# Azure/mmlspark

Hardware: AMD Instinct MI355X
Metric: lightgbm_train_rows_per_sec (higher is better)
Workload: dtype fp32; 1 GPU; model=LightGBMClassifier, rows_per_gpu=10000000, features=100, num_leaves=63, max_bin=255, objective=binary, global_batch=10000000, parallelism=dp1, sync=single rank, categorical=0, matrix=dense

## Files before the change

### mmlspark_amd/models/gbdt/trainer.py

```python
from __future__ import annotations

import heapq
import math
import os
import time
from dataclasses import dataclass, field
from typing import Dict, List, Optional

import numpy as np
import torch

from ...ops import backend
from ...parallel.comm import Comm
from .binning import BinMapper
from .booster import Booster
from .objectives import Objective
from .tree import Tree

NEG_INF = float("-inf")


@dataclass
class TrainConfig:
    num_iterations: int = 100
# ... 231 lines not shown
            order = np.lexsort((present, ratio))
            GL = np.cumsum(g[order], dtype=np.float32)
            HL = np.cumsum(hh[order], dtype=np.float32)
            CL = np.cumsum(c[order], dtype=np.float32)
            G, H, C = GL[-1], HL[-1], CL[-1]

            def sc(Gs, Hs):
                Ga = np.maximum(np.abs(Gs) - np.float32(cfg.lambda_l1),
                                np.float32(0))
                return Ga * Ga / (Hs + np.float32(cfg.lambda_l2)
                                  + np.float32(1e-32))

            gain = sc(GL, HL) + sc(G - GL, H - HL) - sc(
                np.float32(G), np.float32(H))
            valid = ((CL >= cfg.min_data_in_leaf)
                     & (C - CL >= cfg.min_data_in_leaf)
                     & (HL >= cfg.min_sum_hessian_in_leaf)
                     & (H - HL >= cfg.min_sum_hessian_in_leaf))
            gain = np.where(valid, gain, np.float32(NEG_INF))
            gain[-1] = NEG_INF
            k = int(gain.argmax())
            bg = float(gain[k])
            if not np.isfinite(bg):
                continue
            if best is None or bg > best[0]:
                cats = present[order[: k + 1]].tolist()
                best = [bg, int(f), 0, float(GL[k]), float(HL[k]),
                        float(CL[k]), cats]
        return best

    def _best_split(self, hist, feat_mask):
        return self._scan(hist.unsqueeze(0), feat_mask)[0]

    def _partition(self, leaf) -> tuple:
        t0 = time.perf_counter()
        if leaf.cats is not None:
            gq, j = leaf.feat // 4, leaf.feat % 4
            bins = self.binned[gq, leaf.rows.long(), j]
            cats_t = torch.tensor(leaf.cats, dtype=bins.dtype,
                                  device=bins.device)
            mask = torch.isin(bins, cats_t)
            rows_l, rows_r = leaf.rows[mask], leaf.rows[~mask]
        else:
            known = (int(leaf.CL) if (self.fixed
                                      and not self.comm.is_distributed
                                      and leaf.C < 1.6e7)
                     else -1)
            rows_l, rows_r = backend.partition_rows(
                self.binned, leaf.rows, leaf.feat, leaf.bin,
                known_left=known)
        self.stats.partition_s += time.perf_counter() - t0
        return rows_l, rows_r

    def _grow_native(self, rows_root, grad, hess, feat_mask):
        from ...ops import _hip_grower
        cfg = self.cfg
        pg = self.comm.native_group()
        cats_active = [f for f in self.cat_features
                       if feat_mask is None or bool(feat_mask[f])]
        num_mask = feat_mask
        if self.cat_features:
            num_mask = (feat_mask.clone() if feat_mask is not None else
                        torch.ones(self.nf_pad, dtype=torch.bool,
                                   device=self.device))
            num_mask[self.cat_features] = False
        cats_t = (torch.tensor(cats_active, dtype=torch.int64)
                  if cats_active else None)
        t0 = time.perf_counter()
        d = _hip_grower.grow_tree_native(
            self.binned, self.binned_pair, rows_root.contiguous(), grad, hess,
            cfg.max_bin,
            self.nf, self.scale_g, self.scale_h, cfg.lambda_l1, cfg.lambda_l2,
            float(cfg.min_data_in_leaf), cfg.min_sum_hessian_in_leaf,
            cfg.min_gain_to_split, cfg.max_delta_step, cfg.num_leaves,
            cfg.max_depth, num_mask, cats_t, self.cat_smooth, pg,
            self.comm.is_distributed or bool(os.environ.get(
                "MMLSPARK_AMD_FORCE_DIST_GROWER")))
        self.stats.hist_s += time.perf_counter() - t0
        feature = d["feature"].numpy()
        thr_bin = d["thr_bin"].numpy()
        cat_offset = d["cat_offset"].numpy()
        threshold = np.array(
            [float("nan") if cat_offset[i] >= 0 else
             self.bin_mapper.bin_upper_value(int(f), int(b)) if f >= 0 else 0.0
             for i, (f, b) in enumerate(zip(feature, thr_bin))],
            dtype=np.float32)
        tree = Tree(feature, threshold, thr_bin, d["left"].numpy(),
                    d["right"].numpy(), d["value"].numpy(),
                    d["count"].numpy(), d["gain"].numpy(),
                    d["leaf_index"].numpy(), shrinkage=1.0,
                    cat_offset=cat_offset,
                    cat_words=d["cat_words"].numpy().view(np.uint32))
        offs = d["leaf_offsets"].tolist()
        nodes = d["leaf_nodes"].tolist()
        leaves = []
        for i, nid in enumerate(nodes):
            lf = _Leaf(int(nid), d["leaf_rows"][offs[i]:offs[i + 1]], None,
                       0, 0, 0, 0)
            leaves.append(lf)
        self.native_leaves = (d["leaf_rows"], d["leaf_offsets"], nodes)
        return tree, leaves

    native_ok = True
    native_leaves = None

    def grow(self, rows_root: torch.Tensor, grad: torch.Tensor,
             hess: torch.Tensor, feat_mask) -> (Tree, List):
        self.native_leaves = None
        if (self.native_ok and self.fixed and not self.voting
                and not os.environ.get(
                    "MMLSPARK_AMD_NO_NATIVE_GROWER")):
            try:
                from ...ops import _hip_grower
                self.set_scales(grad, hess)
                return self._grow_native(rows_root, grad, hess, feat_mask)
            except ImportError:
                pass
        cfg = self.cfg
        feature, threshold, thr_bin = [], [], []
        left, right, value, count, gain_arr, leaf_idx = [], [], [], [], [], []
        cat_off, cat_words = [], []

        def new_node():
            feature.append(-1)
            threshold.append(0.0)
            thr_bin.append(0)
            left.append(-1)
            right.append(-1)
            value.append(0.0)
            count.append(0.0)
            gain_arr.append(0.0)
            leaf_idx.append(-1)
            cat_off.append(-1)
            return len(feature) - 1

        self.set_scales(grad, hess)
        root_hist = self._hist(rows_root, grad, hess)
        if self.voting:
            t = torch.stack([grad[rows_root.long()].sum(),
                             hess[rows_root.long()].sum(),
                             torch.tensor(float(rows_root.numel()),
                                          device=self.device)])
            self.comm.all_reduce(t)
            G, H, C = float(t[0]), float(t[1]), float(t[2])
        else:
            G, H, C = self._sums(root_hist)
        root = _Leaf(new_node(), rows_root, root_hist, G, H, C, 0)
        (root.gain, root.feat, root.bin, root.GL, root.HL, root.CL,
         root.cats) = self._best_split(root_hist, feat_mask)
        count[root.node_id] = C
        value[root.node_id] = _leaf_output(G, H, cfg)

        heap = [(-root.gain, 0, root)]
        seq = 1
        n_leaves = 1
        final_leaves = [root]

        while n_leaves < cfg.num_leaves and heap:
            ngain, _, leaf = heapq.heappop(heap)
            if -ngain <= cfg.min_gain_to_split or not np.isfinite(-ngain):
                continue
            if cfg.max_depth > 0 and leaf.depth >= cfg.max_depth:
                continue
            final_leaves.remove(leaf)

            rows_l, rows_r = self._partition(leaf)

            GL, HL, CL = leaf.GL, leaf.HL, leaf.CL
# ... 196 lines not shown
            objective.group_sizes = group_sizes

        from .sparse import CsrMatrix, bin_csr, fit_bin_mapper_csr
        self.is_sparse = isinstance(X, CsrMatrix)
        if self.is_sparse:
            if cfg.categorical_features:
                raise ValueError("categorical features need dense input "
                                 "(set matrixType='dense')")
            if cfg.boosting == "dart":
                raise ValueError("dart boosting needs dense input "
                                 "(set matrixType='dense')")
        if binned_cache is not None:
            self.bin_mapper, self.binned = binned_cache
        elif self.is_sparse:
            self.bin_mapper = fit_bin_mapper_csr(
                X, n_bins=cfg.max_bin, comm=comm, seed=cfg.seed,
                sample_size=cfg.bin_sample_count)
            self.binned = bin_csr(X, self.bin_mapper)
        else:
            self.bin_mapper = BinMapper.fit(X, n_bins=cfg.max_bin, comm=comm,
                                            seed=cfg.seed,
                                            sample_size=cfg.bin_sample_count,
                                            categorical=cfg.categorical_features,
                                            max_bin_by_feature=cfg.max_bin_by_feature)
            self.binned = self.bin_mapper.transform(X)

        device, n, K = self.device, self.n, self.K
        if init_booster is not None and init_booster.trees:
            base = torch.from_numpy(init_booster.base_score).to(device)
            self.preds = init_booster.predict_raw(X)
            self.trees: List[Tree] = list(init_booster.trees)
            self.tree_w: List[float] = list(init_booster.tree_weights)
        else:
            base = self._global_init_score()
            if base.numel() < K:
                base = base.expand(K).contiguous()
            self.preds = base.unsqueeze(0).expand(n, K).clone()
            if init_score is not None:
                sc = init_score.to(device).float()
                self.preds += sc.unsqueeze(-1) if sc.dim() == 1 else sc
            self.trees = []
            self.tree_w = []
        self.base = base
        n_global = n
        if comm.is_distributed:
            t = torch.tensor([float(n)], device=device)
            comm.all_reduce(t)
            n_global = int(t[0])
        grower_cls = SparseTreeGrower if self.is_sparse else TreeGrower
        self.grower = grower_cls(self.binned, self.nf, cfg, comm, self.stats,
                                 self.bin_mapper, n_global=n_global)
        self.gen = torch.Generator(device="cpu")
        self.all_rows = torch.arange(n, dtype=torch.int32, device=device)
        self.n_start_trees = len(self.trees)
        self.it = 0

    def _global_init_score(self):
        y, weight, device = self.y, self.weight, self.device
        obj, comm = self.objective, self.comm
        if not self.cfg.boost_from_average:
            return torch.zeros(1, device=device)
        if comm.is_distributed:
            w = weight if weight is not None else torch.ones_like(
                y, dtype=torch.float32)
            sums = torch.stack([(y.float() * w).sum(), w.sum()]).to(device)
            comm.all_reduce(sums)
            mean = sums[0] / sums[1].clamp_min(1e-12)
            if obj.name == "binary":
                p = mean.clamp(1e-6, 1 - 1e-6)
                sig = getattr(obj, "sigmoid", 1.0)
                return (torch.log(p / (1 - p)) / sig).reshape(1)
            if obj.name in ("regression", "regression_l2"):
                return mean.reshape(1)
            if obj.name in ("poisson", "tweedie"):
                return torch.log(mean.clamp_min(1e-8)).reshape(1)
            s0 = obj.init_score(y, weight).to(device).float()
            comm.all_reduce(s0)
            return s0 / comm.world_size
        return obj.init_score(y, weight).to(device)

    def step(self):
        cfg, gen, K, device = self.cfg, self.gen, self.K, self.device
        trees, tree_w, preds = self.trees, self.tree_w, self.preds
        it = self.it
        rf_mode = cfg.boosting == "rf"
        dart_mode = cfg.boosting == "dart"
        goss_mode = cfg.boosting == "goss"

        t0 = time.perf_counter()
        dropped = []
        if dart_mode and trees[self.n_start_trees:]:
            gen.manual_seed(cfg.seed * 7919 + it)
            if float(torch.rand(1, generator=gen)) >= cfg.skip_drop:
                cand = list(range(self.n_start_trees, len(trees)))
                if cfg.uniform_drop:
                    pdrop = torch.full((len(cand),), cfg.drop_rate)
                else:
                    tw = torch.tensor([abs(tree_w[t]) for t in cand])
                    pdrop = (cfg.drop_rate * len(cand)
                             * tw / tw.sum().clamp_min(1e-12)).clamp(0, 1)
                mask = torch.rand(len(cand), generator=gen) < pdrop
                dropped = [cand[i] for i in range(len(cand)) if bool(mask[i])]
                dropped = dropped[: cfg.max_drop]
        if dropped:
            drop_contrib = torch.zeros_like(preds)
            for t in dropped:
                k = (t - self.n_start_trees) % K
                drop_contrib[:, k] += tree_w[t] * predict_tree_binned(
                    trees[t], self.binned, device)
            preds_used = preds - drop_contrib
        else:
            preds_used = preds
        if rf_mode:
            preds_used = self.base.unsqueeze(0).expand(self.n, K)
        grad, hess = self.objective.grad_hess(preds_used, self.y, self.weight)
        self.stats.grad_s += time.perf_counter() - t0

        gen.manual_seed(cfg.bagging_seed * 104729 + it * 31 + self.comm.rank)
        if goss_mode and it >= 1:
            rows_root = _goss_sample(grad, hess, cfg, gen)
        elif (cfg.pos_bagging_fraction < 1.0 or cfg.neg_bagging_fraction < 1.0) \
                and cfg.bagging_freq > 0 and it % cfg.bagging_freq == 0:
            pos = (self.y > 0).cpu()
            keep = torch.rand(self.n, generator=gen) < torch.where(
                pos, torch.tensor(cfg.pos_bagging_fraction),
                torch.tensor(cfg.neg_bagging_fraction))
            rows_root = keep.nonzero(as_tuple=True)[0].to(
                device, torch.int32).sort().values
            if rows_root.numel() == 0:
                rows_root = self.all_rows
        elif (cfg.bagging_freq > 0 and cfg.bagging_fraction < 1.0
              and it % cfg.bagging_freq == 0) or rf_mode:
            frac = cfg.bagging_fraction if cfg.bagging_fraction < 1.0 else 0.632
            m = max(1, int(frac * self.n))
            perm = torch.randperm(self.n, generator=gen)[:m].to(device)
            rows_root = perm.to(torch.int32).sort().values
        else:
            rows_root = self.all_rows

        feat_mask = None
        if cfg.feature_fraction < 1.0:
            gen_f = torch.Generator(device="cpu")
            gen_f.manual_seed(cfg.seed * 524287 + it)
            kf = max(1, int(cfg.feature_fraction * self.nf))
            sel = torch.randperm(self.nf, generator=gen_f)[:kf]
            feat_mask = torch.zeros(self.grower.nf_pad, dtype=torch.bool,
                                    device=device)
            feat_mask[sel.to(device)] = True

        new_trees = []
        for k in range(K):
            tree, leaves = self.grower.grow(rows_root, grad[:, k].contiguous(),
                                            hess[:, k].contiguous(), feat_mask)
            tree.shrinkage = 1.0 if rf_mode else cfg.learning_rate
            if not rf_mode:
                t0 = time.perf_counter()
                live = [lf for lf in leaves if lf.rows.numel()]
                native = self.grower.native_leaves
                if (native is not None and not dropped
                        and preds.is_cuda and preds.dtype == torch.float32):
                    from ...ops import _hip_grower
                    leaf_rows, leaf_offsets, nodes = native
                    vals = torch.tensor(
                        [float(tree.value[nid]) * tree.shrinkage
                         for nid in nodes], dtype=torch.float32,
                        device=device)
                    _hip_grower.apply_leaf_values(preds[:, k], leaf_rows,
                                                  leaf_offsets, vals)
                elif live:
                    all_rows = torch.cat([lf.rows for lf in live]).long()
                    sizes = [lf.rows.numel() for lf in live]
                    vals = torch.tensor(
                        [float(tree.value[lf.node_id]) * tree.shrinkage
                         for lf in live], device=device)
                    expanded = torch.repeat_interleave(
                        vals, torch.tensor(sizes, device=device))
                    preds[:, k].index_add_(0, all_rows, expanded)
                self.stats.partition_s += time.perf_counter() - t0
            new_trees.append(tree)

        if dropped:
            kdrop = len(dropped)
            if cfg.xgboost_dart_mode:
                factor = kdrop / (kdrop + cfg.learning_rate)
                new_scale = cfg.learning_rate / (kdrop + cfg.learning_rate)
            else:
                factor = kdrop / (kdrop + 1.0)
                new_scale = 1.0 / (kdrop + 1.0)
            for t in dropped:
                k = (t - self.n_start_trees) % K
                delta = (factor - 1.0) * tree_w[t]
                preds[:, k] += delta * predict_tree_binned(trees[t], self.binned,
                                                           device)
                tree_w[t] *= factor
            for k, tr in enumerate(new_trees):
                excess = (1.0 - new_scale) * tr.shrinkage
                preds[:, k] -= excess * predict_tree_binned(tr, self.binned, device)
                tr.shrinkage *= new_scale

        for tr in new_trees:
            trees.append(tr)
            tree_w.append(1.0)
        self.stats.iterations += 1
        self.it += 1

    def booster(self) -> Booster:
        tw = list(self.tree_w)
        if self.cfg.boosting == "rf" and self.stats.iterations:
            tw = [1.0 / self.stats.iterations] * len(tw)
        return Booster(list(self.trees), self.objective.name, self.K,
                       self.base.cpu().numpy(), self.nf, self.feature_names,
                       self.bin_mapper,
                       sigmoid=getattr(self.objective, "sigmoid", 1.0),
# ... 103 lines not shown
```

### mmlspark_amd/ops/hip/gbdt_grower.cpp

```cpp
#include <torch/extension.h>
#include <torch/csrc/distributed/c10d/ProcessGroup.hpp>
#include <c10/hip/HIPGuard.h>
#include <c10/hip/HIPStream.h>
#include <hip/hip_runtime.h>

#include <algorithm>
#include <cmath>
#include <cstdlib>
#include <memory>
#include <mutex>
#include <numeric>
#include <queue>
#include <vector>

extern "C" {
void launch_arena_gather(const void*, long, const float*, const float*,
                         const int*, long, int, double, double, void*, void*,
                         int*, hipStream_t);
void launch_partition_arena(const void*, const void*, const int*, void*,
                            void*, int*, long, int, long, long, int, int,
                            const unsigned*, int*, int*, long, int,
                            hipStream_t);
void launch_hist_pair_range(const void*, const void*, long, long, long,
                            long long*, int, int, int, const int*, int, long,
                            int, int, int, hipStream_t);
void launch_sibling_scan(const long long*, const long long*, long long*, int,
                         long, int, float, float, float, float, long,
                         const bool*, float*, double, double, hipStream_t);
void launch_apply_leaf_values(float*, long, const int*, const long*, int,
                              const float*, long, hipStream_t);
}

static hipStream_t grower_stream() {
  return c10::hip::getCurrentHIPStream().stream();
}

namespace {

constexpr int kMaxGrowerStreams = 3;
constexpr int kDefaultGrowerStreams = 3;

std::vector<c10::hip::HIPStream> grower_streams(int n) {
  auto cur = c10::hip::getCurrentHIPStream();
  std::vector<c10::hip::HIPStream> out{cur};
  if (n <= 1) return out;
  static std::mutex mu;
  static std::vector<std::vector<c10::hip::HIPStream>> side;
  std::lock_guard<std::mutex> lock(mu);
  const size_t dev = (size_t)cur.device_index();
  if (side.size() <= dev) side.resize(dev + 1);
  while ((int)side[dev].size() < kMaxGrowerStreams - 1)
    side[dev].push_back(
        c10::hip::getStreamFromPool(false, cur.device_index()));
  for (int i = 0; i + 1 < n; ++i) out.push_back(side[dev][i]);
  return out;
}

int grower_streams_from_env() {
  const char* e = std::getenv("MMLSPARK_AMD_GROWER_STREAMS");
  if (!e || !*e) return kDefaultGrowerStreams;
  char* end = nullptr;
  const long v = std::strtol(e, &end, 10);
  TORCH_CHECK(*end == '\0' && v >= 1 && v <= kMaxGrowerStreams,
              "MMLSPARK_AMD_GROWER_STREAMS must be 1..", kMaxGrowerStreams,
              ", got '", e, "'");
  return (int)v;
}

long hist_env(const char* name, long unset) {
  const char* e = std::getenv(name);
  if (!e || !*e) return unset;
  char* end = nullptr;
  const long v = std::strtol(e, &end, 10);
  TORCH_CHECK(*end == '\0' && v >= 0, name,
              " must be a non-negative integer, got '", e, "'");
  return v;
}

int hist_threads(long arg = 0) {
  const long v = arg != 0 ? arg : hist_env("MMLSPARK_AMD_HIST_THREADS", 0);
  TORCH_CHECK(v == 0 || v == 256 || v == 512 || v == 1024,
              "threads / MMLSPARK_AMD_HIST_THREADS must be 0, 256, 512 or "
              "1024, got ", v);
  return (int)v;
}

int hist_order(long arg = -1) {
  const long v = arg != -1 ? arg : hist_env("MMLSPARK_AMD_HIST_ORDER", -1);
  TORCH_CHECK(v >= -1 && v <= 1,
              "order / MMLSPARK_AMD_HIST_ORDER must be 0 or 1, got ", v);
  return (int)v;
}

int hist_layout(long arg = -1) {
  const long v = arg != -1 ? arg : hist_env("MMLSPARK_AMD_HIST_LAYOUT", -1);
  TORCH_CHECK(v >= -1 && v <= 2,
              "layout / MMLSPARK_AMD_HIST_LAYOUT must be 0, 1 or 2, got ", v);
  return (int)v;
}

struct GrowCtx {
  long n_arena;
  int n_bins;
  int npairs;
  int tail_bytes;
  torch::Tensor pair[2];
  torch::Tensor ghq[2];
  torch::Tensor rowid[2];
  long nf;
  double scale_g, scale_h;
  double l1, l2, min_data, min_hess, min_gain;
  int num_leaves, max_depth;
  torch::Tensor feat_mask;
  c10::intrusive_ptr<c10d::ProcessGroup> pg;
  bool has_reduce;
  bool distributed;
  std::vector<int> cat_feats;
  double cat_smooth = 10.0;
  torch::Tensor cat_idx_dev;
  std::vector<c10::hip::HIPStream> streams;
  size_t next_stream = 0;
  torch::Tensor scratch[kMaxGrowerStreams];
  torch::Tensor total[kMaxGrowerStreams];
  torch::Tensor slab_zero, slab_raw;
  long slab_used_zero = 0, slab_used_raw = 0;
};

struct SplitJob {
  torch::Tensor hist_l, hist_r;
  torch::Tensor scan_host;
  torch::Tensor nl_host;
  torch::Tensor cat_host;
  torch::Tensor bits_host;
  torch::Tensor bits_dev;
  long nl_known = -1;
  hipEvent_t ev = nullptr;

  ~SplitJob() {
    if (ev) {
      (void)hipEventSynchronize(ev);
      (void)hipEventDestroy(ev);
    }
  }
};

struct LeafCand {
  double gain = 0;
  long seq = 0;
  int node_id = 0;
  int depth = 0;
  long lo = 0, hi = 0;
  int buf = 0;
  torch::Tensor hist;
  double G = 0, H = 0, C = 0;
  double GL = 0, HL = 0, CL = 0;
  int feat = -1, bin = 0;
  std::vector<int> cats;
  std::shared_ptr<SplitJob> job;
};

using CandPtr = std::shared_ptr<LeafCand>;

struct CandCmp {
  bool operator()(const CandPtr& a, const CandPtr& b) const {
    if (a->gain != b->gain) return a->gain < b->gain;
    return a->seq > b->seq;
  }
};

torch::Tensor hist_slot(GrowCtx& ctx, bool zeroed) {
  torch::Tensor& slab = zeroed ? ctx.slab_zero : ctx.slab_raw;
  long& used = zeroed ? ctx.slab_used_zero : ctx.slab_used_raw;
  if (used < slab.size(0)) return slab.select(0, used++);
  auto opt = ctx.pair[0].options();
  return zeroed ? torch::zeros({ctx.npairs * 8, ctx.n_bins, 3}, opt)
                : torch::empty({ctx.npairs * 8, ctx.n_bins, 3}, opt);
}

torch::Tensor build_hist(GrowCtx& ctx, int buf, long lo, long m,
                         const int* nl_dev = nullptr, int side = -1) {
  auto hist = hist_slot(ctx, true);
  launch_hist_pair_range(
      ctx.pair[buf].data_ptr(), ctx.ghq[buf].data_ptr(), ctx.n_arena, lo, m,
      (long long*)hist.data_ptr<int64_t>(), ctx.n_bins, ctx.npairs,
      ctx.tail_bytes, nl_dev, side, 0, hist_threads(), hist_order(),
      hist_layout(), grower_stream());
  if (ctx.has_reduce) {
    std::vector<at::Tensor> v{hist};
    ctx.pg->allreduce(v)->wait();
  }
  return hist;
}

void launch_scan_async(GrowCtx& ctx, const torch::Tensor& parent,
                       const torch::Tensor& small, torch::Tensor big,
                       bool small_is_left, SplitJob& job) {
  const long nh = parent.defined() ? 2 : 1;
  const long nf_pad = small.size(0);
  auto records = torch::empty(
      {nh, nf_pad, 6},
      torch::TensorOptions().dtype(torch::kFloat32).device(small.device()));
  const bool* mask = ctx.feat_mask.defined()
                         ? ctx.feat_mask.data_ptr<bool>() : nullptr;
  launch_sibling_scan(
      parent.defined() ? (const long long*)parent.data_ptr<int64_t>()
                       : nullptr,
      (const long long*)small.data_ptr<int64_t>(),
      big.defined() ? (long long*)big.data_ptr<int64_t>() : nullptr,
      small_is_left ? 1 : 0, nf_pad, ctx.n_bins, (float)ctx.l1, (float)ctx.l2,
      (float)ctx.min_data, (float)ctx.min_hess, ctx.nf, mask,
      records.data_ptr<float>(), 1.0 / ctx.scale_g, 1.0 / ctx.scale_h,
      grower_stream());
  job.scan_host = torch::empty({nh, nf_pad, 6}, torch::TensorOptions()
                                                    .dtype(torch::kFloat32)
                                                    .pinned_memory(true));
  (void)hipMemcpyAsync(job.scan_host.data_ptr<float>(),
                       records.data_ptr<float>(),
                       nh * nf_pad * 6 * sizeof(float), hipMemcpyDeviceToHost,
                       grower_stream());
  if (!ctx.cat_feats.empty()) {
    const long ncat = (long)ctx.cat_feats.size();
    const size_t per_hist = (size_t)ncat * ctx.n_bins * 3;
    job.cat_host = torch::empty({nh, ncat, (long)ctx.n_bins, 3},
                                torch::TensorOptions()
                                    .dtype(torch::kInt64)
                                    .pinned_memory(true));
    for (long h = 0; h < nh; ++h) {
      const torch::Tensor& src = (h == 0) == small_is_left ? small : big;
      auto cat_rows = src.index_select(0, ctx.cat_idx_dev).contiguous();
      (void)hipMemcpyAsync(job.cat_host.data_ptr<int64_t>() + h * per_hist,
                           cat_rows.data_ptr<int64_t>(),
                           per_hist * sizeof(int64_t), hipMemcpyDeviceToHost,
                           grower_stream());
    }
  }
  (void)hipEventCreateWithFlags(&job.ev, hipEventDisableTiming);
  (void)hipEventRecord(job.ev, grower_stream());
}

struct CatBest {
  float gain = -INFINITY;
  int feat = -1;
  float GL = 0, HL = 0, CL = 0;
  std::vector<int> cats;
};

CatBest cat_scan_host(const GrowCtx& ctx, const int64_t* hist) {
  CatBest best;
  const int nb = ctx.n_bins;
  const double inv_g = 1.0 / ctx.scale_g, inv_h = 1.0 / ctx.scale_h;
  for (size_t ci = 0; ci < ctx.cat_feats.size(); ++ci) {
    const int64_t* h = hist + ci * (size_t)nb * 3;
    std::vector<int> present;
    for (int b = 0; b < nb; ++b)
      if (h[b * 3 + 2] > 0) present.push_back(b);
    const int m = (int)present.size();
    if (m < 2) continue;
    std::vector<float> g(m), hh(m), c(m), ratio(m);
    for (int i = 0; i < m; ++i) {
      const int b = present[i];
      g[i] = (float)((double)h[b * 3 + 0] * inv_g);
      hh[i] = (float)((double)h[b * 3 + 1] * inv_h);
      c[i] = (float)h[b * 3 + 2];
      ratio[i] = g[i] / (hh[i] + (float)ctx.cat_smooth);
    }
    std::vector<int> order(m);
    std::iota(order.begin(), order.end(), 0);
    std::stable_sort(order.begin(), order.end(), [&](int x, int y) {
      if (ratio[x] != ratio[y]) return ratio[x] < ratio[y];
      return present[x] < present[y];
    });
    std::vector<float> GL(m), HL(m), CL(m);
    float ag = 0.f, ah = 0.f, ac = 0.f;
    for (int i = 0; i < m; ++i) {
      ag += g[order[i]]; ah += hh[order[i]]; ac += c[order[i]];
      GL[i] = ag; HL[i] = ah; CL[i] = ac;
    }
    const float G = GL[m - 1], H = HL[m - 1], C = CL[m - 1];
    auto sc = [&](float Gs, float Hs) {
      const float Ga = std::max(std::fabs(Gs) - (float)ctx.l1, 0.0f);
      return Ga * Ga / (Hs + (float)ctx.l2 + 1e-32f);
    };
    const float scGH = sc(G, H);
    int bi = -1;
    float bg = -INFINITY;
    for (int i = 0; i < m - 1; ++i) {
      const bool valid = CL[i] >= (float)ctx.min_data
          && (C - CL[i]) >= (float)ctx.min_data
          && HL[i] >= (float)ctx.min_hess
          && (H - HL[i]) >= (float)ctx.min_hess;
      const float gain = valid
          ? sc(GL[i], HL[i]) + sc(G - GL[i], H - HL[i]) - scGH
          : -INFINITY;
      if (gain > bg) { bg = gain; bi = i; }
    }
    if (bi < 0 || !std::isfinite(bg)) continue;
    if (best.feat < 0 || bg > best.gain) {
      best.gain = bg;
      best.feat = ctx.cat_feats[ci];
      best.GL = GL[bi]; best.HL = HL[bi]; best.CL = CL[bi];
      best.cats.assign(order.begin(), order.begin() + bi + 1);
      for (auto& v : best.cats) v = present[v];
    }
  }
  return best;
}

void resolve_best(const GrowCtx& ctx, SplitJob& job, int hi, LeafCand& c) {
  auto rec = job.scan_host.accessor<float, 3>()[hi];
  long bf = 0;
  float best = -INFINITY;
  for (long f = 0; f < rec.size(0); ++f)
    if (rec[f][0] > best) { best = rec[f][0]; bf = f; }
  auto a = rec[bf];
  c.gain = a[0]; c.feat = (int)a[1]; c.bin = (int)a[2];
  c.GL = a[3]; c.HL = a[4]; c.CL = a[5];
  c.cats.clear();
  if (!ctx.cat_feats.empty()) {
    const size_t stride =
        ctx.cat_feats.size() * (size_t)ctx.n_bins * 3;
    CatBest cb = cat_scan_host(
        ctx, job.cat_host.data_ptr<int64_t>() + (size_t)hi * stride);
    if (cb.feat >= 0 && (double)cb.gain > c.gain) {
      c.gain = (double)cb.gain; c.feat = cb.feat; c.bin = 0;
      c.GL = (double)cb.GL; c.HL = (double)cb.HL; c.CL = (double)cb.CL;
      c.cats = std::move(cb.cats);
    }
  }
}

void launch_job(GrowCtx& ctx, LeafCand& leaf) {
  const size_t si = ctx.next_stream;
  ctx.next_stream = (ctx.next_stream + 1) % ctx.streams.size();
  c10::hip::HIPStreamGuard guard(ctx.streams[si]);
  int* const scratch = ctx.scratch[si].data_ptr<int>();
  int* const total = ctx.total[si].data_ptr<int>();
  auto job = std::make_shared<SplitJob>();
  const long m = leaf.hi - leaf.lo;
  const int src = leaf.buf, dst = leaf.buf ^ 1;
  const unsigned* cat_bits = nullptr;
  if (!leaf.cats.empty()) {
    job->bits_host = torch::zeros({8}, torch::TensorOptions()
                                           .dtype(torch::kInt32)
                                           .pinned_memory(true));
    unsigned* wb = (unsigned*)job->bits_host.data_ptr<int>();
    for (int b : leaf.cats) wb[b >> 5] |= (1u << (b & 31));
    job->bits_dev = torch::empty({8}, ctx.rowid[0].options()
                                          .dtype(torch::kInt32));
    (void)hipMemcpyAsync(job->bits_dev.data_ptr<int>(), wb,
                         8 * sizeof(int), hipMemcpyHostToDevice,
                         grower_stream());
    cat_bits = (const unsigned*)job->bits_dev.data_ptr<int>();
  }
  launch_partition_arena(
      ctx.pair[src].data_ptr(), ctx.ghq[src].data_ptr(),
      ctx.rowid[src].data_ptr<int>(), ctx.pair[dst].data_ptr(),
      ctx.ghq[dst].data_ptr(), ctx.rowid[dst].data_ptr<int>(), ctx.n_arena,
      ctx.npairs, leaf.lo, m, leaf.feat, leaf.bin, cat_bits,
      scratch, total, 0, 0, grower_stream());

  const double CL = leaf.CL, CR = leaf.C - leaf.CL;
  const bool left_small = CL <= CR;
  torch::Tensor hist_small;
  if (!ctx.distributed && leaf.C < 1.6e7) {
    job->nl_known = (long)leaf.CL;
    const long lo_s = left_small ? leaf.lo : leaf.lo + job->nl_known;
    const long m_s = left_small ? job->nl_known : m - job->nl_known;
    hist_small = build_hist(ctx, dst, lo_s, m_s);
  } else {
    hist_small = build_hist(ctx, dst, leaf.lo, m, total, left_small ? 0 : 1);
    job->nl_host = torch::empty({1}, torch::TensorOptions()
                                         .dtype(torch::kInt32)
                                         .pinned_memory(true));
    (void)hipMemcpyAsync(job->nl_host.data_ptr<int>(), total, sizeof(int),
                         hipMemcpyDeviceToHost, grower_stream());
  }
  auto hist_big = hist_slot(ctx, false);
  job->hist_l = left_small ? hist_small : hist_big;
  job->hist_r = left_small ? hist_big : hist_small;
  launch_scan_async(ctx, leaf.hist, hist_small, hist_big, left_small, *job);
  leaf.job = job;
}

double leaf_output(double G, double H, double l1, double l2,
                   double max_delta) {
  double g = std::abs(G) - l1;
  if (g <= 0) return 0.0;
  double denom = H + l2;
  if (denom <= 0) return 0.0;
  double w = -std::copysign(g, G) / denom;
  if (max_delta > 0) w = std::clamp(w, -max_delta, max_delta);
  return w;
}

bool splittable(const GrowCtx& ctx, const LeafCand& c) {
  if (!(c.gain > ctx.min_gain) || !std::isfinite(c.gain)) return false;
  if (ctx.max_depth > 0 && c.depth >= ctx.max_depth) return false;
  return true;
}

}

py::dict grow_tree_native(torch::Tensor binned, torch::Tensor binned_pair,
                          torch::Tensor rows_root,
                          torch::Tensor grad, torch::Tensor hess,
                          long n_bins, long nf, double scale_g, double scale_h,
                          double l1, double l2, double min_data,
                          double min_hess, double min_gain, double max_delta,
                          long num_leaves, long max_depth,
                          c10::optional<torch::Tensor> feat_mask,
                          c10::optional<torch::Tensor> cat_feats,
                          double cat_smooth,
                          py::object process_group, bool distributed) {
  GrowCtx ctx;
  const long n_full = binned_pair.size(1);
  ctx.n_arena = rows_root.numel();
  ctx.n_bins = (int)n_bins;
  ctx.npairs = (int)binned_pair.size(0);
  ctx.tail_bytes = (int)(binned.size(0) * 4 - (ctx.npairs - 1) * 8);
  ctx.nf = nf;
  ctx.scale_g = scale_g;
  ctx.scale_h = scale_h;
  ctx.l1 = l1; ctx.l2 = l2;
  ctx.min_data = min_data; ctx.min_hess = min_hess; ctx.min_gain = min_gain;
  ctx.num_leaves = (int)num_leaves;
  ctx.max_depth = (int)max_depth;
  if (feat_mask.has_value()) ctx.feat_mask = *feat_mask;
  if (cat_feats.has_value() && cat_feats->numel() > 0) {
    auto cf = cat_feats->to(torch::kInt64).contiguous().cpu();
    auto acc = cf.accessor<int64_t, 1>();
    for (long i = 0; i < cf.numel(); ++i)
      ctx.cat_feats.push_back((int)acc[i]);
    ctx.cat_idx_dev = cf.to(binned.device());
    ctx.cat_smooth = cat_smooth;
  }
  if (!process_group.is_none()) {
    ctx.pg = process_group.cast<c10::intrusive_ptr<c10d::ProcessGroup>>();
  }
  ctx.has_reduce = ctx.pg && ctx.pg->getSize() > 1;
  ctx.distributed = distributed;
  ctx.streams = grower_streams(ctx.has_reduce ? 1 : grower_streams_from_env());
  (void)hist_threads();
  (void)hist_order();
  (void)hist_layout();

  py::gil_scoped_release nogil;

  for (size_t s = 0; s < ctx.streams.size(); ++s) {
    ctx.scratch[s] =
        torch::empty({4096}, rows_root.options().dtype(torch::kInt32));
    ctx.total[s] = torch::zeros({1}, rows_root.options().dtype(torch::kInt32));
  }
  auto i64d = rows_root.options().dtype(torch::kInt64);
  const long slot_bytes = (long)ctx.npairs * 8 * ctx.n_bins * 3 * 8;
  const long slots = std::min<long>(ctx.num_leaves + 2,
                                    std::max<long>(1, (1l << 30) / slot_bytes));
  ctx.slab_zero = torch::zeros({slots, ctx.npairs * 8, ctx.n_bins, 3}, i64d);
  ctx.slab_raw = torch::empty({slots, ctx.npairs * 8, ctx.n_bins, 3}, i64d);
  for (int b = 0; b < 2; ++b) {
    ctx.pair[b] = torch::empty({ctx.npairs, ctx.n_arena}, i64d);
    ctx.ghq[b] = torch::empty({ctx.n_arena, 2}, i64d);
    ctx.rowid[b] = torch::empty({ctx.n_arena},
                                rows_root.options().dtype(torch::kInt32));
  }
  launch_arena_gather(binned_pair.data_ptr(), n_full,
                      grad.data_ptr<float>(), hess.data_ptr<float>(),
                      rows_root.data_ptr<int>(), ctx.n_arena, ctx.npairs,
                      ctx.scale_g, ctx.scale_h, ctx.pair[0].data_ptr(),
                      ctx.ghq[0].data_ptr(), ctx.rowid[0].data_ptr<int>(),
                      grower_stream());

  std::vector<int> feature_, thr_bin_, left_, right_, leaf_idx_;
  std::vector<int> cat_off_, cat_words_;
  std::vector<float> value_, count_, gain_;
  auto new_node = [&]() {
    feature_.push_back(-1); thr_bin_.push_back(0); left_.push_back(-1);
    right_.push_back(-1); value_.push_back(0.f); count_.push_back(0.f);
    gain_.push_back(0.f); leaf_idx_.push_back(-1); cat_off_.push_back(-1);
    return (int)feature_.size() - 1;
  };

  auto root_hist = build_hist(ctx, 0, 0, ctx.n_arena);
  auto sums = root_hist.select(0, 0).sum(0).to(torch::kCPU);
  auto sa = sums.accessor<int64_t, 1>();
  const double G0 = (double)sa[0] / scale_g;
  const double H0 = (double)sa[1] / scale_h;
  const double C0 = (double)sa[2];

  auto root = std::make_shared<LeafCand>();
  root->node_id = new_node();
  root->lo = 0; root->hi = ctx.n_arena; root->buf = 0;
  root->hist = root_hist;
  root->G = G0; root->H = H0; root->C = C0;
  {
    SplitJob j;
    launch_scan_async(ctx, torch::Tensor(), root_hist, torch::Tensor(), true,
                      j);
    (void)hipEventSynchronize(j.ev);
    resolve_best(ctx, j, 0, *root);
  }
  count_[root->node_id] = (float)C0;
  value_[root->node_id] = (float)leaf_output(G0, H0, l1, l2, max_delta);

  std::priority_queue<CandPtr, std::vector<CandPtr>, CandCmp> heap;
  std::vector<CandPtr> finals;
  heap.push(root);
  finals.push_back(root);
  long seq = 1;
  int n_leaves = 1;

  while (n_leaves < ctx.num_leaves && !heap.empty()) {
    CandPtr leaf = heap.top();
    heap.pop();
    if (!splittable(ctx, *leaf)) continue;
    for (size_t i = 0; i < finals.size(); ++i)
      if (finals[i]->node_id == leaf->node_id) {
        finals.erase(finals.begin() + i);
        break;
      }

    if (!leaf->job) launch_job(ctx, *leaf);
    if (n_leaves + 1 < ctx.num_leaves && !heap.empty()) {
      CandPtr nxt = heap.top();
      if (!nxt->job && splittable(ctx, *nxt)) launch_job(ctx, *nxt);
      if (n_leaves + 2 < ctx.num_leaves && heap.size() >= 2) {
        heap.pop();
        CandPtr nxt2 = heap.top();
        heap.push(nxt);
        if (!nxt2->job && splittable(ctx, *nxt2)) launch_job(ctx, *nxt2);
      }
    }

    SplitJob& job = *leaf->job;
    (void)hipEventSynchronize(job.ev);
    const long m_parent = leaf->hi - leaf->lo;
    const long nl = job.nl_known >= 0
                        ? job.nl_known
                        : (long)job.nl_host.data_ptr<int>()[0];

    const double GL = leaf->GL, HL = leaf->HL, CL = leaf->CL;
    const double GR = leaf->G - GL, HR = leaf->H - HL, CR = leaf->C - CL;
    const int nid = leaf->node_id;
    feature_[nid] = leaf->feat;
    thr_bin_[nid] = leaf->bin;
    gain_[nid] = (float)leaf->gain;
    if (!leaf->cats.empty()) {
      unsigned words[8] = {0};
      for (int b : leaf->cats) words[b >> 5] |= (1u << (b & 31));
      cat_off_[nid] = (int)(cat_words_.size() / 8);
      for (int w = 0; w < 8; ++w) cat_words_.push_back((int)words[w]);
    }
    const int lid = new_node();
    const int rid = new_node();
    left_[nid] = lid;
    right_[nid] = rid;
    count_[lid] = (float)CL;
    count_[rid] = (float)CR;
    value_[lid] = (float)leaf_output(GL, HL, l1, l2, max_delta);
    value_[rid] = (float)leaf_output(GR, HR, l1, l2, max_delta);

    auto lc = std::make_shared<LeafCand>();
    auto rc = std::make_shared<LeafCand>();
    lc->node_id = lid; rc->node_id = rid;
    lc->depth = rc->depth = leaf->depth + 1;
    lc->buf = rc->buf = leaf->buf ^ 1;
    lc->lo = leaf->lo; lc->hi = leaf->lo + nl;
    rc->lo = leaf->lo + nl; rc->hi = leaf->lo + m_parent;
    lc->hist = job.hist_l; rc->hist = job.hist_r;
    lc->G = GL; lc->H = HL; lc->C = CL;
    rc->G = GR; rc->H = HR; rc->C = CR;
    resolve_best(ctx, job, 0, *lc);
    resolve_best(ctx, job, 1, *rc);
    lc->seq = seq++;
    rc->seq = seq++;
    leaf->job.reset();
    leaf->hist = torch::Tensor();
    heap.push(lc);
    heap.push(rc);
    finals.push_back(lc);
    finals.push_back(rc);
    n_leaves += 1;
  }

  for (size_t s = 1; s < ctx.streams.size(); ++s) {
    hipEvent_t ev = nullptr;
    (void)hipEventCreateWithFlags(&ev, hipEventDisableTiming);
    (void)hipEventRecord(ev, ctx.streams[s].stream());
    (void)hipStreamWaitEvent(grower_stream(), ev, 0);
    (void)hipEventDestroy(ev);
  }

  std::sort(finals.begin(), finals.end(),
            [](const CandPtr& a, const CandPtr& b) {
              return a->node_id < b->node_id;
            });
  std::vector<torch::Tensor> segs;
  std::vector<int64_t> seg_nodes;
  for (size_t i = 0; i < finals.size(); ++i) {
    leaf_idx_[finals[i]->node_id] = (int)i;
    segs.push_back(ctx.rowid[finals[i]->buf].slice(0, finals[i]->lo,
                                                   finals[i]->hi));
    seg_nodes.push_back(finals[i]->node_id);
  }
  auto leaf_rows = segs.empty()
                       ? torch::empty({0}, rows_root.options())
                       : torch::cat(segs);
  std::vector<int64_t> offs(1, 0);
  for (auto& s : segs) offs.push_back(offs.back() + s.numel());

  py::gil_scoped_acquire gil;
  auto i32 = torch::TensorOptions().dtype(torch::kInt32);
  auto f32 = torch::TensorOptions().dtype(torch::kFloat32);
  py::dict d;
  d["feature"] = torch::tensor(feature_, i32);
  d["thr_bin"] = torch::tensor(thr_bin_, i32);
  d["left"] = torch::tensor(left_, i32);
  d["right"] = torch::tensor(right_, i32);
  d["value"] = torch::tensor(value_, f32);
  d["count"] = torch::tensor(count_, f32);
  d["gain"] = torch::tensor(gain_, f32);
  d["leaf_index"] = torch::tensor(leaf_idx_, i32);
  d["leaf_rows"] = leaf_rows;
  d["leaf_offsets"] = torch::tensor(offs, torch::kInt64);
  d["leaf_nodes"] = torch::tensor(seg_nodes, torch::kInt64);
  d["cat_offset"] = torch::tensor(cat_off_, i32);
  d["cat_words"] = cat_words_.empty()
                       ? torch::zeros({0}, i32)
                       : torch::tensor(cat_words_, i32);
  return d;
}

void allreduce_native(py::object process_group, torch::Tensor t) {
  auto pg = process_group.cast<c10::intrusive_ptr<c10d::ProcessGroup>>();
  py::gil_scoped_release nogil;
  std::vector<at::Tensor> v{t};
  pg->allreduce(v)->wait();
}

void apply_leaf_values(torch::Tensor preds_col, torch::Tensor leaf_rows,
                       torch::Tensor leaf_offsets, torch::Tensor values) {
  TORCH_CHECK(preds_col.is_cuda() && preds_col.dim() == 1 &&
              preds_col.scalar_type() == torch::kFloat32,
              "preds_col: 1-D f32 device tensor");
  TORCH_CHECK(leaf_rows.is_cuda() && leaf_rows.is_contiguous() &&
              leaf_rows.scalar_type() == torch::kInt32,
              "leaf_rows: contiguous i32 device tensor");
  TORCH_CHECK(values.is_cuda() && values.is_contiguous() &&
              values.scalar_type() == torch::kFloat32,
              "values: contiguous f32 device tensor");
  TORCH_CHECK(leaf_offsets.scalar_type() == torch::kInt64 &&
              leaf_offsets.numel() == values.numel() + 1,
              "leaf_offsets: i64 of n_leaves + 1");
  auto offs_cpu = leaf_offsets.cpu();
  const int64_t* oc = offs_cpu.data_ptr<int64_t>();
  const long n_leaves = values.numel();
  TORCH_CHECK(oc[0] == 0 && oc[n_leaves] == leaf_rows.numel(),
              "leaf_offsets must span leaf_rows");
  for (long l = 0; l < n_leaves; ++l)
    TORCH_CHECK(oc[l] <= oc[l + 1], "leaf_offsets must be non-decreasing");
  auto offs = leaf_offsets.to(preds_col.device()).contiguous();
  launch_apply_leaf_values(preds_col.data_ptr<float>(), preds_col.stride(0),
                           leaf_rows.data_ptr<int>(),
                           (const long*)offs.data_ptr<int64_t>(),
                           (int)n_leaves, values.data_ptr<float>(),
                           leaf_rows.numel(), grower_stream());
}

torch::Tensor partition_arena(torch::Tensor pair_src, torch::Tensor ghq_src,
                              torch::Tensor rowid_src, torch::Tensor pair_dst,
                              torch::Tensor ghq_dst, torch::Tensor rowid_dst,
                              long lo, long m, long feature, long thr,
                              c10::optional<torch::Tensor> cat_bits,
                              long chunk, long plane_groups) {
  const long n_arena = pair_src.size(1);
  const long npairs = pair_src.size(0);
  TORCH_CHECK(pair_src.is_cuda() && pair_src.is_contiguous() &&
              pair_src.scalar_type() == torch::kInt64 &&
              pair_dst.is_contiguous() && pair_dst.sizes() == pair_src.sizes(),
              "pair planes: contiguous (npairs, n_arena) i64");
  TORCH_CHECK(ghq_src.is_contiguous() && ghq_dst.is_contiguous() &&
              ghq_src.numel() == 2 * n_arena && ghq_dst.numel() == 2 * n_arena,
// ... 12 lines not shown
  }
  auto i32 = rowid_src.options().dtype(torch::kInt32);
  auto scratch = torch::empty({4096}, i32);
  auto total = torch::zeros({1}, i32);
  launch_partition_arena(pair_src.data_ptr(), ghq_src.data_ptr(),
                         rowid_src.data_ptr<int>(), pair_dst.data_ptr(),
                         ghq_dst.data_ptr(), rowid_dst.data_ptr<int>(),
                         n_arena, (int)npairs, lo, m, (int)feature, (int)thr,
                         bits, scratch.data_ptr<int>(), total.data_ptr<int>(),
                         chunk, (int)plane_groups, grower_stream());
  return total;
}

void hist_pair_range(torch::Tensor pair, torch::Tensor ghq, long lo, long m,
                     torch::Tensor hist, long n_bins, long tail_bytes,
                     c10::optional<torch::Tensor> nl_dev, long side,
                     long chunk, long threads, long order, long layout) {
  TORCH_CHECK(pair.is_cuda() && pair.is_contiguous() && pair.dim() == 2 &&
              pair.scalar_type() == torch::kInt64,
              "pair planes: contiguous (npairs, n_arena) i64");
  const long n_arena = pair.size(1);
  const long npairs = pair.size(0);
  TORCH_CHECK(ghq.is_cuda() && ghq.is_contiguous() &&
              ghq.scalar_type() == torch::kInt64 &&
              ghq.numel() == 2 * n_arena,
              "ghq: contiguous (n_arena, 2) i64");
  TORCH_CHECK(lo >= 0 && m >= 0 && lo + m <= n_arena, "range out of bounds");
  TORCH_CHECK(n_bins >= 1 && n_bins <= 256, "n_bins must be 1..256");
  TORCH_CHECK(tail_bytes >= 1 && tail_bytes <= 8, "tail_bytes must be 1..8");
  TORCH_CHECK(hist.is_cuda() && hist.is_contiguous() &&
              hist.scalar_type() == torch::kInt64 &&
              hist.numel() == npairs * 8 * n_bins * 3,
              "hist: contiguous (npairs * 8, n_bins, 3) i64");
  TORCH_CHECK(side >= -1 && side <= 1, "side must be -1, 0 or 1");
  TORCH_CHECK(chunk >= 0, "chunk must be >= 0");
  const int threads_r = hist_threads(threads);
  const int order_r = hist_order(order);
  const int layout_r = hist_layout(layout);
  const int* nl = nullptr;
  if (side >= 0) {
    TORCH_CHECK(nl_dev.has_value() && nl_dev->is_cuda() &&
                nl_dev->scalar_type() == torch::kInt32 &&
                nl_dev->numel() == 1, "nl_dev: (1,) i32 device");
    nl = nl_dev->data_ptr<int>();
  }
  launch_hist_pair_range(pair.data_ptr(), ghq.data_ptr(), n_arena, lo, m,
                         (long long*)hist.data_ptr<int64_t>(), (int)n_bins,
                         (int)npairs, (int)tail_bytes, nl, (int)side, chunk,
                         threads_r, order_r, layout_r, grower_stream());
}

PYBIND11_MODULE(TORCH_EXTENSION_NAME, m) {
  m.def("grow_tree_native", &grow_tree_native,
        "native leaf-wise GBDT tree growth (numeric features, arena mode)");
  m.def("apply_leaf_values", &apply_leaf_values,
        "preds_col[leaf_rows] += per-leaf value, one kernel");
  m.def("partition_arena", &partition_arena,
        "arena stable partition (count + fused scatter)", py::arg("pair_src"),
        py::arg("ghq_src"), py::arg("rowid_src"), py::arg("pair_dst"),
        py::arg("ghq_dst"), py::arg("rowid_dst"), py::arg("lo"), py::arg("m"),
        py::arg("feature"), py::arg("thr"), py::arg("cat_bits") = py::none(),
        py::arg("chunk") = 0, py::arg("plane_groups") = 0);
  m.def("hist_pair_range", &hist_pair_range,
        "range-mode arena histogram, accumulated into hist", py::arg("pair"),
        py::arg("ghq"), py::arg("lo"), py::arg("m"), py::arg("hist"),
        py::arg("n_bins"), py::arg("tail_bytes"),
        py::arg("nl_dev") = py::none(), py::arg("side") = -1,
        py::arg("chunk") = 0, py::arg("threads") = 0, py::arg("order") = -1,
        py::arg("layout") = -1);
  m.def("allreduce_native", &allreduce_native,
        "GIL-free c10d all_reduce through the same C++ path as the grower");
}
```

Baseline: 1.142 billion rows/s.

## Skip root arena gather, fold root sums into scan, apply leaf values in grower

When all rows are used, the root level reads bin planes directly from the original binned tensor instead of gathering them into the arena. The first partition then writes into buffer 1. Root gradient sums now come from a pinned copy made alongside the split scan, so one host wait replaces two. Leaf-value application to predictions moves inside the native grower, and the per-tree Python leaf list and per-split threshold lookups are made lazy or cached on the host. Together these cut a full-arena copy per tree, a sync, and Python overhead, at the cost of more buffer-index bookkeeping.

```diff
diff --git a/mmlspark_amd/models/gbdt/trainer.py b/mmlspark_amd/models/gbdt/trainer.py
--- a/mmlspark_amd/models/gbdt/trainer.py
+++ b/mmlspark_amd/models/gbdt/trainer.py
@@ -307,7 +307,7 @@
         self.stats.partition_s += time.perf_counter() - t0
         return rows_l, rows_r
 
-    def _grow_native(self, rows_root, grad, hess, feat_mask):
+    def _grow_native(self, rows_root, grad, hess, feat_mask, update=None):
         from ...ops import _hip_grower
         cfg = self.cfg
         pg = self.comm.native_group()
@@ -321,6 +321,9 @@
             num_mask[self.cat_features] = False
         cats_t = (torch.tensor(cats_active, dtype=torch.int64)
                   if cats_active else None)
+        identity = (self.identity_rows is not None
+                    and rows_root is self.identity_rows)
+        preds_col, shrinkage = update if update is not None else (None, 1.0)
         t0 = time.perf_counter()
         d = _hip_grower.grow_tree_native(
             self.binned, self.binned_pair, rows_root.contiguous(), grad, hess,
@@ -330,14 +333,21 @@
             cfg.min_gain_to_split, cfg.max_delta_step, cfg.num_leaves,
             cfg.max_depth, num_mask, cats_t, self.cat_smooth, pg,
             self.comm.is_distributed or bool(os.environ.get(
-                "MMLSPARK_AMD_FORCE_DIST_GROWER")))
+                "MMLSPARK_AMD_FORCE_DIST_GROWER")),
+            rows_identity=identity, preds_col=preds_col, shrinkage=shrinkage)
         self.stats.hist_s += time.perf_counter() - t0
         feature = d["feature"].numpy()
         thr_bin = d["thr_bin"].numpy()
         cat_offset = d["cat_offset"].numpy()
+        if self._upper_bounds_host is None:
+            self._upper_bounds_host = \
+                self.bin_mapper.upper_bounds.detach().cpu().numpy()
+        ub = self._upper_bounds_host
+        last_bin = self.bin_mapper.n_bins - 1
         threshold = np.array(
             [float("nan") if cat_offset[i] >= 0 else
-             self.bin_mapper.bin_upper_value(int(f), int(b)) if f >= 0 else 0.0
+             (float("inf") if b >= last_bin else float(ub[f, b]))
+             if f >= 0 else 0.0
              for i, (f, b) in enumerate(zip(feature, thr_bin))],
             dtype=np.float32)
         tree = Tree(feature, threshold, thr_bin, d["left"].numpy(),
@@ -346,29 +356,35 @@
                     d["leaf_index"].numpy(), shrinkage=1.0,
                     cat_offset=cat_offset,
                     cat_words=d["cat_words"].numpy().view(np.uint32))
-        offs = d["leaf_offsets"].tolist()
         nodes = d["leaf_nodes"].tolist()
-        leaves = []
-        for i, nid in enumerate(nodes):
-            lf = _Leaf(int(nid), d["leaf_rows"][offs[i]:offs[i + 1]], None,
-                       0, 0, 0, 0)
-            leaves.append(lf)
         self.native_leaves = (d["leaf_rows"], d["leaf_offsets"], nodes)
-        return tree, leaves
+        self.native_applied = bool(int(d["preds_applied"][0]))
+        return tree, None
+
+    def native_leaf_list(self):
+        leaf_rows, leaf_offsets, nodes = self.native_leaves
+        offs = leaf_offsets.tolist()
+        return [_Leaf(int(nid), leaf_rows[offs[i]:offs[i + 1]], None,
+                      0, 0, 0, 0) for i, nid in enumerate(nodes)]
 
     native_ok = True
     native_leaves = None
+    native_applied = False
+    identity_rows = None
+    _upper_bounds_host = None
 
     def grow(self, rows_root: torch.Tensor, grad: torch.Tensor,
-             hess: torch.Tensor, feat_mask) -> (Tree, List):
+             hess: torch.Tensor, feat_mask, update=None) -> (Tree, List):
         self.native_leaves = None
+        self.native_applied = False
         if (self.native_ok and self.fixed and not self.voting
                 and not os.environ.get(
                     "MMLSPARK_AMD_NO_NATIVE_GROWER")):
             try:
                 from ...ops import _hip_grower
                 self.set_scales(grad, hess)
-                return self._grow_native(rows_root, grad, hess, feat_mask)
+                return self._grow_native(rows_root, grad, hess, feat_mask,
+                                         update)
             except ImportError:
                 pass
         cfg = self.cfg
@@ -671,6 +687,7 @@
                                  self.bin_mapper, n_global=n_global)
         self.gen = torch.Generator(device="cpu")
         self.all_rows = torch.arange(n, dtype=torch.int32, device=device)
+        self.grower.identity_rows = self.all_rows
         self.n_start_trees = len(self.trees)
         self.it = 0
 
@@ -769,15 +786,22 @@
 
         new_trees = []
         for k in range(K):
-            tree, leaves = self.grower.grow(rows_root, grad[:, k].contiguous(),
-                                            hess[:, k].contiguous(), feat_mask)
+            fused = (not rf_mode and not dropped and preds.is_cuda
+                     and preds.dtype == torch.float32)
+            tree, leaves = self.grower.grow(
+                rows_root, grad[:, k].contiguous(), hess[:, k].contiguous(),
+                feat_mask,
+                update=(preds[:, k], cfg.learning_rate) if fused else None)
             tree.shrinkage = 1.0 if rf_mode else cfg.learning_rate
             if not rf_mode:
                 t0 = time.perf_counter()
-                live = [lf for lf in leaves if lf.rows.numel()]
                 native = self.grower.native_leaves
-                if (native is not None and not dropped
-                        and preds.is_cuda and preds.dtype == torch.float32):
+                if leaves is None and not (native is not None and fused):
+                    leaves = self.grower.native_leaf_list()
+                live = [lf for lf in leaves or () if lf.rows.numel()]
+                if self.grower.native_applied:
+                    pass
+                elif native is not None and fused:
                     from ...ops import _hip_grower
                     leaf_rows, leaf_offsets, nodes = native
                     vals = torch.tensor(
diff --git a/mmlspark_amd/ops/hip/gbdt_grower.cpp b/mmlspark_amd/ops/hip/gbdt_grower.cpp
--- a/mmlspark_amd/ops/hip/gbdt_grower.cpp
+++ b/mmlspark_amd/ops/hip/gbdt_grower.cpp
@@ -67,6 +67,14 @@
   return (int)v;
 }
 
+bool grower_switch(const char* name) {
+  const char* e = std::getenv(name);
+  if (!e || !*e) return true;
+  TORCH_CHECK((e[0] == '0' || e[0] == '1') && e[1] == '\0', name,
+              " must be 0 or 1, got '", e, "'");
+  return e[0] == '1';
+}
+
 long hist_env(const char* name, long unset) {
   const char* e = std::getenv(name);
   if (!e || !*e) return unset;
@@ -105,6 +113,7 @@
   int npairs;
   int tail_bytes;
   torch::Tensor pair[2];
+  const void* root_pair = nullptr;
   torch::Tensor ghq[2];
   torch::Tensor rowid[2];
   long nf;
@@ -126,6 +135,14 @@
   long slab_used_zero = 0, slab_used_raw = 0;
 };
 
+constexpr int kRootBuf = 2;
+
+const void* pair_of(const GrowCtx& ctx, int buf) {
+  return buf == kRootBuf ? ctx.root_pair : ctx.pair[buf].data_ptr();
+}
+int small_buf(int buf) { return buf == kRootBuf ? 0 : buf; }
+int child_buf(int buf) { return buf == kRootBuf ? 1 : buf ^ 1; }
+
 struct SplitJob {
   torch::Tensor hist_l, hist_r;
   torch::Tensor scan_host;
@@ -133,6 +150,7 @@
   torch::Tensor cat_host;
   torch::Tensor bits_host;
   torch::Tensor bits_dev;
+  torch::Tensor row0_host;
   long nl_known = -1;
   hipEvent_t ev = nullptr;
 
@@ -181,7 +199,7 @@
                          const int* nl_dev = nullptr, int side = -1) {
   auto hist = hist_slot(ctx, true);
   launch_hist_pair_range(
-      ctx.pair[buf].data_ptr(), ctx.ghq[buf].data_ptr(), ctx.n_arena, lo, m,
+      pair_of(ctx, buf), ctx.ghq[small_buf(buf)].data_ptr(), ctx.n_arena, lo, m,
       (long long*)hist.data_ptr<int64_t>(), ctx.n_bins, ctx.npairs,
       ctx.tail_bytes, nl_dev, side, 0, hist_threads(), hist_order(),
       hist_layout(), grower_stream());
@@ -194,7 +212,7 @@
 
 void launch_scan_async(GrowCtx& ctx, const torch::Tensor& parent,
                        const torch::Tensor& small, torch::Tensor big,
-                       bool small_is_left, SplitJob& job) {
+                       bool small_is_left, SplitJob& job, bool row0 = false) {
   const long nh = parent.defined() ? 2 : 1;
   const long nf_pad = small.size(0);
   auto records = torch::empty(
@@ -233,6 +251,15 @@
                            per_hist * sizeof(int64_t), hipMemcpyDeviceToHost,
                            grower_stream());
     }
+  }
+  if (row0) {
+    job.row0_host = torch::empty({(long)ctx.n_bins, 3}, torch::TensorOptions()
+                                                            .dtype(torch::kInt64)
+                                                            .pinned_memory(true));
+    (void)hipMemcpyAsync(job.row0_host.data_ptr<int64_t>(),
+                         small.data_ptr<int64_t>(),
+                         (size_t)ctx.n_bins * 3 * sizeof(int64_t),
+                         hipMemcpyDeviceToHost, grower_stream());
   }
   (void)hipEventCreateWithFlags(&job.ev, hipEventDisableTiming);
   (void)hipEventRecord(job.ev, grower_stream());
@@ -337,7 +364,7 @@
   int* const total = ctx.total[si].data_ptr<int>();
   auto job = std::make_shared<SplitJob>();
   const long m = leaf.hi - leaf.lo;
-  const int src = leaf.buf, dst = leaf.buf ^ 1;
+  const int src = leaf.buf, dst = child_buf(leaf.buf);
   const unsigned* cat_bits = nullptr;
   if (!leaf.cats.empty()) {
     job->bits_host = torch::zeros({8}, torch::TensorOptions()
@@ -353,8 +380,8 @@
     cat_bits = (const unsigned*)job->bits_dev.data_ptr<int>();
   }
   launch_partition_arena(
-      ctx.pair[src].data_ptr(), ctx.ghq[src].data_ptr(),
-      ctx.rowid[src].data_ptr<int>(), ctx.pair[dst].data_ptr(),
+      pair_of(ctx, src), ctx.ghq[small_buf(src)].data_ptr(),
+      ctx.rowid[small_buf(src)].data_ptr<int>(), ctx.pair[dst].data_ptr(),
       ctx.ghq[dst].data_ptr(), ctx.rowid[dst].data_ptr<int>(), ctx.n_arena,
       ctx.npairs, leaf.lo, m, leaf.feat, leaf.bin, cat_bits,
       scratch, total, 0, 0, grower_stream());
@@ -411,10 +438,29 @@
                           c10::optional<torch::Tensor> feat_mask,
                           c10::optional<torch::Tensor> cat_feats,
                           double cat_smooth,
-                          py::object process_group, bool distributed) {
+                          py::object process_group, bool distributed,
+                          bool rows_identity,
+                          c10::optional<torch::Tensor> preds_col,
+                          double shrinkage) {
   GrowCtx ctx;
   const long n_full = binned_pair.size(1);
   ctx.n_arena = rows_root.numel();
+  const bool root_static =
+      grower_switch("MMLSPARK_AMD_GROWER_ROOT_STATIC") && rows_identity;
+  const bool root_one_wait = grower_switch("MMLSPARK_AMD_GROWER_ROOT_ONE_WAIT");
+  const bool apply_here =
+      grower_switch("MMLSPARK_AMD_GROWER_APPLY") && preds_col.has_value();
+  if (rows_identity)
+    TORCH_CHECK(ctx.n_arena == n_full && binned_pair.is_contiguous() &&
+                binned_pair.scalar_type() == torch::kInt64,
+                "rows_identity needs rows_root to be all ", n_full,
+                " rows and contiguous i64 bin planes, got ", ctx.n_arena,
+                " rows");
+  if (preds_col.has_value())
+    TORCH_CHECK(preds_col->is_cuda() && preds_col->dim() == 1 &&
+                preds_col->scalar_type() == torch::kFloat32 &&
+                preds_col->size(0) >= n_full,
+                "preds_col: 1-D f32 device tensor over all rows");
   ctx.n_bins = (int)n_bins;
   ctx.npairs = (int)binned_pair.size(0);
   ctx.tail_bytes = (int)(binned.size(0) * 4 - (ctx.npairs - 1) * 8);
@@ -463,9 +509,11 @@
     ctx.rowid[b] = torch::empty({ctx.n_arena},
                                 rows_root.options().dtype(torch::kInt32));
   }
+  if (root_static) ctx.root_pair = binned_pair.data_ptr();
   launch_arena_gather(binned_pair.data_ptr(), n_full,
                       grad.data_ptr<float>(), hess.data_ptr<float>(),
-                      rows_root.data_ptr<int>(), ctx.n_arena, ctx.npairs,
+                      rows_root.data_ptr<int>(), ctx.n_arena,
+                      root_static ? 0 : ctx.npairs,
                       ctx.scale_g, ctx.scale_h, ctx.pair[0].data_ptr(),
                       ctx.ghq[0].data_ptr(), ctx.rowid[0].data_ptr<int>(),
                       grower_stream());
@@ -480,25 +528,36 @@
     return (int)feature_.size() - 1;
   };
 
-  auto root_hist = build_hist(ctx, 0, 0, ctx.n_arena);
-  auto sums = root_hist.select(0, 0).sum(0).to(torch::kCPU);
-  auto sa = sums.accessor<int64_t, 1>();
-  const double G0 = (double)sa[0] / scale_g;
-  const double H0 = (double)sa[1] / scale_h;
-  const double C0 = (double)sa[2];
-
+  const int root_buf = root_static ? kRootBuf : 0;
+  auto root_hist = build_hist(ctx, root_buf, 0, ctx.n_arena);
   auto root = std::make_shared<LeafCand>();
   root->node_id = new_node();
-  root->lo = 0; root->hi = ctx.n_arena; root->buf = 0;
+  root->lo = 0; root->hi = ctx.n_arena; root->buf = root_buf;
   root->hist = root_hist;
-  root->G = G0; root->H = H0; root->C = C0;
-  {
+  int64_t s0[3] = {0, 0, 0};
+  if (root_one_wait) {
+    SplitJob j;
+    launch_scan_async(ctx, torch::Tensor(), root_hist, torch::Tensor(), true,
+                      j, true);
+    (void)hipEventSynchronize(j.ev);
+    const int64_t* r = j.row0_host.data_ptr<int64_t>();
+    for (int b = 0; b < ctx.n_bins; ++b)
+      for (int c = 0; c < 3; ++c) s0[c] += r[b * 3 + c];
+    resolve_best(ctx, j, 0, *root);
+  } else {
+    auto sums = root_hist.select(0, 0).sum(0).to(torch::kCPU);
+    auto sa = sums.accessor<int64_t, 1>();
+    for (int c = 0; c < 3; ++c) s0[c] = sa[c];
     SplitJob j;
     launch_scan_async(ctx, torch::Tensor(), root_hist, torch::Tensor(), true,
                       j);
     (void)hipEventSynchronize(j.ev);
     resolve_best(ctx, j, 0, *root);
   }
+  const double G0 = (double)s0[0] / scale_g;
+  const double H0 = (double)s0[1] / scale_h;
+  const double C0 = (double)s0[2];
+  root->G = G0; root->H = H0; root->C = C0;
   count_[root->node_id] = (float)C0;
   value_[root->node_id] = (float)leaf_output(G0, H0, l1, l2, max_delta);
 
@@ -563,7 +622,7 @@
     auto rc = std::make_shared<LeafCand>();
     lc->node_id = lid; rc->node_id = rid;
     lc->depth = rc->depth = leaf->depth + 1;
-    lc->buf = rc->buf = leaf->buf ^ 1;
+    lc->buf = rc->buf = child_buf(leaf->buf);
     lc->lo = leaf->lo; lc->hi = leaf->lo + nl;
     rc->lo = leaf->lo + nl; rc->hi = leaf->lo + m_parent;
     lc->hist = job.hist_l; rc->hist = job.hist_r;
@@ -598,8 +657,8 @@
   std::vector<int64_t> seg_nodes;
   for (size_t i = 0; i < finals.size(); ++i) {
     leaf_idx_[finals[i]->node_id] = (int)i;
-    segs.push_back(ctx.rowid[finals[i]->buf].slice(0, finals[i]->lo,
-                                                   finals[i]->hi));
+    segs.push_back(ctx.rowid[small_buf(finals[i]->buf)].slice(
+        0, finals[i]->lo, finals[i]->hi));
     seg_nodes.push_back(finals[i]->node_id);
   }
   auto leaf_rows = segs.empty()
@@ -607,6 +666,25 @@
                        : torch::cat(segs);
   std::vector<int64_t> offs(1, 0);
   for (auto& s : segs) offs.push_back(offs.back() + s.numel());
+
+  const bool applied = apply_here && leaf_rows.numel() > 0;
+  if (applied) {
+    const long nl = (long)segs.size();
+    auto pin = torch::TensorOptions().pinned_memory(true);
+    auto offs_h = torch::empty({nl + 1}, pin.dtype(torch::kInt64));
+    auto vals_h = torch::empty({nl}, pin.dtype(torch::kFloat32));
+    std::copy(offs.begin(), offs.end(), offs_h.data_ptr<int64_t>());
+    for (long i = 0; i < nl; ++i)
+      vals_h.data_ptr<float>()[i] =
+          (float)((double)value_[seg_nodes[i]] * shrinkage);
+    auto offs_d = offs_h.to(leaf_rows.device(), true);
+    auto vals_d = vals_h.to(leaf_rows.device(), true);
+    launch_apply_leaf_values(preds_col->data_ptr<float>(),
+                             preds_col->stride(0), leaf_rows.data_ptr<int>(),
+                             (const long*)offs_d.data_ptr<int64_t>(), (int)nl,
+                             vals_d.data_ptr<float>(), leaf_rows.numel(),
+                             grower_stream());
+  }
 
   py::gil_scoped_acquire gil;
   auto i32 = torch::TensorOptions().dtype(torch::kInt32);
@@ -627,6 +705,7 @@
   d["cat_words"] = cat_words_.empty()
                        ? torch::zeros({0}, i32)
                        : torch::tensor(cat_words_, i32);
+  d["preds_applied"] = torch::full({1}, applied ? 1 : 0, i32);
   return d;
 }
 
@@ -745,7 +824,15 @@
 
 PYBIND11_MODULE(TORCH_EXTENSION_NAME, m) {
   m.def("grow_tree_native", &grow_tree_native,
-        "native leaf-wise GBDT tree growth (numeric features, arena mode)");
+        "native leaf-wise GBDT tree growth (arena mode)", py::arg("binned"),
+        py::arg("binned_pair"), py::arg("rows_root"), py::arg("grad"),
+        py::arg("hess"), py::arg("n_bins"), py::arg("nf"), py::arg("scale_g"),
+        py::arg("scale_h"), py::arg("l1"), py::arg("l2"), py::arg("min_data"),
+        py::arg("min_hess"), py::arg("min_gain"), py::arg("max_delta"),
+        py::arg("num_leaves"), py::arg("max_depth"), py::arg("feat_mask"),
+        py::arg("cat_feats"), py::arg("cat_smooth"), py::arg("process_group"),
+        py::arg("distributed"), py::arg("rows_identity") = false,
+        py::arg("preds_col") = py::none(), py::arg("shrinkage") = 1.0);
   m.def("apply_leaf_values", &apply_leaf_values,
         "preds_col[leaf_rows] += per-leaf value, one kernel");
   m.def("partition_arena", &partition_arena,
```

After: 1.403 billion rows/s, median of 6. 1.23x the previous value.
